# SEP-software/zfp-par

Hardware: AMD Instinct MI355X
Metric: GB/s uncompressed, 3D float32 fixed-rate encode, device-resident (higher is better)
Workload: dtype f32; 1 GPU; 1024^3 float32 fixed-rate 16 zfp_compress per GPU (BASELINE configs[1]); field=smooth, mode=rate, param=16, stream_bytes_per_gpu=2147483648, parallelism=1 independent z-slab chunks, one per GPU

## Files before the change

zfp-par_amd/csrc/hip/block3.h:

```cpp
#pragma once

#include "codec_dev.h"

namespace zfp_amd {

template <typename S>
__device__ __forceinline__ void pad_line(S* v, int b, int s, int n)
{
  if (n <= 1) v[b + s] = v[b];
  if (n <= 2) v[b + 2 * s] = v[b + s];
  if (n <= 3) v[b + 3 * s] = v[b];
}

struct FastDiv {
  uint32_t m, s1, s2;
};

__host__ __device__ inline FastDiv make_fastdiv(uint32_t d)
{
  if (d == 0)
    d = 1;
  uint32_t l = 0;
  while (l < 32 && (1ull << l) < d)
    l++;
// ... 82 lines not shown
#ifndef ZFP_NT_LOAD
#define ZFP_NT_LOAD 1
#endif
#ifndef ZFP_NT_STORE
#define ZFP_NT_STORE 1
#endif
template <typename S, int N>
__device__ __forceinline__ Vec16<S, N> load16(const S* p)
{
#if ZFP_NT_LOAD && defined(__HIP_DEVICE_COMPILE__)
  typedef uint32_t u4 __attribute__((ext_vector_type(4)));
  const u4 x = __builtin_nontemporal_load(reinterpret_cast<const u4*>(p));
  Vec16<S, N> r;
  __builtin_memcpy(&r, &x, 16);
  return r;
#else
  return *reinterpret_cast<const Vec16<S, N>*>(p);
#endif
}

template <typename S, int N>
__device__ __forceinline__ void store16(S* p, const Vec16<S, N>& q)
{
#if ZFP_NT_STORE && defined(__HIP_DEVICE_COMPILE__)
  typedef uint32_t u4 __attribute__((ext_vector_type(4)));
  u4 x;
  __builtin_memcpy(&x, &q, 16);
  __builtin_nontemporal_store(x, reinterpret_cast<u4*>(p));
#else
  *reinterpret_cast<Vec16<S, N>*>(p) = q;
#endif
}

template <typename S, bool VEC, bool NOPART = false>
__device__ __forceinline__ void gather3(S (&v)[64], const S* __restrict__ base, const Geometry& g, const BlockPos& p)
{
  const S* o = base + p.off;
  const int64_t sx = g.s[0], sy = g.s[1], sz = g.s[2];
  if (NOPART || p.full) {
#pragma unroll
    for (int k = 0; k < 4; k++)
#pragma unroll
      for (int j = 0; j < 4; j++) {
        const S* r = o + j * sy + k * sz;
        if (VEC) {
          if constexpr (sizeof(S) == 4) {
            const Vec16<S, 4> q = load16<S, 4>(r);
#pragma unroll
            for (int i = 0; i < 4; i++)
              v[16 * k + 4 * j + i] = q.v[i];
          } else {
            const Vec16<S, 2> q0 = load16<S, 2>(r);
            const Vec16<S, 2> q1 = load16<S, 2>(r + 2);
            v[16 * k + 4 * j + 0] = q0.v[0];
            v[16 * k + 4 * j + 1] = q0.v[1];
            v[16 * k + 4 * j + 2] = q1.v[0];
            v[16 * k + 4 * j + 3] = q1.v[1];
          }
        } else {
#pragma unroll
          for (int i = 0; i < 4; i++)
            v[16 * k + 4 * j + i] = r[i * sx];
        }
      }
  } else {
    const int cx = p.cnt[0], cy = p.cnt[1], cz = p.cnt[2];
#pragma unroll
    for (int k = 0; k < 4; k++)
#pragma unroll
      for (int j = 0; j < 4; j++)
#pragma unroll
        for (int i = 0; i < 4; i++)
          v[16 * k + 4 * j + i] = (i < cx && j < cy && k < cz) ? o[i * sx + j * sy + k * sz] : (S)0;
#pragma unroll
    for (int k = 0; k < 4; k++)
#pragma unroll
      for (int j = 0; j < 4; j++)
        if (k < cz && j < cy) pad_line(v, 16 * k + 4 * j, 1, cx);
#pragma unroll
    for (int k = 0; k < 4; k++)
#pragma unroll
      for (int i = 0; i < 4; i++)
        if (k < cz) pad_line(v, 16 * k + i, 4, cy);
#pragma unroll
    for (int j = 0; j < 4; j++)
#pragma unroll
      for (int i = 0; i < 4; i++)
        pad_line(v, 4 * j + i, 16, cz);
  }
}

template <typename S, bool VEC>
__device__ __forceinline__ void scatter3(const S (&v)[64], S* __restrict__ base, const Geometry& g, const BlockPos& p)
{
  S* o = base + p.off;
  const int64_t sx = g.s[0], sy = g.s[1], sz = g.s[2];
  if (p.full) {
#pragma unroll
    for (int k = 0; k < 4; k++)
#pragma unroll
      for (int j = 0; j < 4; j++) {
        S* r = o + j * sy + k * sz;
        if (VEC) {
          if constexpr (sizeof(S) == 4) {
            Vec16<S, 4> q;
#pragma unroll
            for (int i = 0; i < 4; i++)
              q.v[i] = v[16 * k + 4 * j + i];
            store16<S, 4>(r, q);
          } else {
            Vec16<S, 2> q0, q1;
            q0.v[0] = v[16 * k + 4 * j + 0];
            q0.v[1] = v[16 * k + 4 * j + 1];
            q1.v[0] = v[16 * k + 4 * j + 2];
            q1.v[1] = v[16 * k + 4 * j + 3];
            store16<S, 2>(r, q0);
            store16<S, 2>(r + 2, q1);
          }
        } else {
#pragma unroll
          for (int i = 0; i < 4; i++)
            r[i * sx] = v[16 * k + 4 * j + i];
        }
      }
  } else {
    const int cx = p.cnt[0], cy = p.cnt[1], cz = p.cnt[2];
#pragma unroll
    for (int k = 0; k < 4; k++)
#pragma unroll
      for (int j = 0; j < 4; j++)
#pragma unroll
        for (int i = 0; i < 4; i++)
          if (i < cx && j < cy && k < cz) o[i * sx + j * sy + k * sz] = v[16 * k + 4 * j + i];
  }
}

template <bool P3 = true>
__device__ __forceinline__ void planes_from_coeffs(uint32_t (&Pl)[32], uint32_t (&Ph)[32], const int32_t (&q)[64])
{
#pragma unroll
  for (int i = 0; i < 32; i++) {
    Pl[i] = nb_planes((uint32_t)q[P3 ? kPerm3[i] : i] + 0xaaaaaaaau);
    Ph[i] = nb_planes((uint32_t)q[P3 ? kPerm3[i + 32] : i + 32] + 0xaaaaaaaau);
  }
  transpose32_nb(Pl);
  transpose32_nb(Ph);
}

#ifndef ZFP_NARROW_HI
#define ZFP_NARROW_HI 1
#endif

template <bool P3 = true, int B = 32, int E = 64>
__device__ __forceinline__ bool high_half_narrow(const int32_t (&q)[64])
{
  uint32_t acc = 0;
#pragma unroll
  for (int i = B; i < E; i++)
    acc = __builtin_amdgcn_bitop3_b32(acc, (uint32_t)q[P3 ? kPerm3[i] : i] + 0xaaaaaaaau, 0xaaaaaaaau, 0xf6);
  return acc < 256u;
}

template <bool P3 = true>
__device__ __forceinline__ void planes_high_narrow(uint32_t (&Ph)[32], const int32_t (&q)[64])
{
  uint32_t W[8];
#pragma unroll
  for (int j = 0; j < 8; j++) {
    uint32_t a[4];
#pragma unroll
    for (int b = 0; b < 4; b++)
      a[b] = nb_planes((uint32_t)q[P3 ? kPerm3[32 + 8 * b + j] : 32 + 8 * b + j] + 0xaaaaaaaau);
    const uint32_t t0 = __builtin_amdgcn_perm(a[1], a[0], 0x05010400u);
    const uint32_t t1 = __builtin_amdgcn_perm(a[3], a[2], 0x05010400u);
    W[j] = __builtin_amdgcn_perm(t1, t0, 0x05040100u);
  }
  transpose8x4_nb(W);
#pragma unroll
  for (int k = 0; k < 32; k++)
    Ph[k] = k < 8 ? W[k] : 0u;
}

template <bool P3 = true>
__device__ __forceinline__ void planes_high_full(uint32_t (&Ph)[32], const int32_t (&q)[64])
{
#pragma unroll
  for (int i = 0; i < 32; i++)
    Ph[i] = nb_planes((uint32_t)q[P3 ? kPerm3[i + 32] : i + 32] + 0xaaaaaaaau);
  transpose32_nb(Ph);
}

template <bool P3 = true>
__device__ __forceinline__ void planes_low(uint32_t (&Pl)[32], const int32_t (&q)[64])
{
#pragma unroll
  for (int i = 0; i < 32; i++)
    Pl[i] = nb_planes((uint32_t)q[P3 ? kPerm3[i] : i] + 0xaaaaaaaau);
  transpose32_nb(Pl);
}

template <bool P3 = true>
__device__ __forceinline__ void planes_from_coeffs_narrow(uint32_t (&Pl)[32], uint32_t (&Ph)[32],
                                                          const int32_t (&q)[64])
{
  planes_low<P3>(Pl, q);
  planes_high_narrow<P3>(Ph, q);
}

template <bool P3 = true>
__device__ __forceinline__ void planes_from_coeffs_auto(uint32_t (&Pl)[32], uint32_t (&Ph)[32],
                                                        const int32_t (&q)[64])
{
  planes_low<P3>(Pl, q);
  pin_registers(Pl);
  if (ZFP_NARROW_HI && __builtin_amdgcn_ballot_w64(!high_half_narrow<P3, 32, 40>(q)) == 0 &&
      __builtin_amdgcn_ballot_w64(!high_half_narrow<P3, 40, 64>(q)) == 0)
    planes_high_narrow<P3>(Ph, q);
  else
    planes_high_full<P3>(Ph, q);
}

template <bool P3 = true>
__device__ __forceinline__ void planes_from_coeffs(uint32_t (&Pl)[64], uint32_t (&Ph)[64], const int64_t (&q)[64],
                                                   bool need_low)
{
  uint32_t a[32], b[32];
#pragma unroll
  for (int i = 0; i < 32; i++) {
    uint64_t u0 = nb_planes((uint64_t)q[P3 ? kPerm3[i] : i] + 0xaaaaaaaaaaaaaaaaull);
    uint64_t u1 = nb_planes((uint64_t)q[P3 ? kPerm3[i + 32] : i + 32] + 0xaaaaaaaaaaaaaaaaull);
    a[i] = (uint32_t)(u0 >> 32);
    b[i] = (uint32_t)(u1 >> 32);
  }
  transpose32_nb(a);
  transpose32_nb(b);
#pragma unroll
  for (int k = 0; k < 32; k++) {
    Pl[32 + k] = a[k];
    Ph[32 + k] = b[k];
  }
  if (__any(need_low)) {
#pragma unroll
    for (int i = 0; i < 32; i++) {
      uint64_t u0 = nb_planes((uint64_t)q[P3 ? kPerm3[i] : i] + 0xaaaaaaaaaaaaaaaaull);
      uint64_t u1 = nb_planes((uint64_t)q[P3 ? kPerm3[i + 32] : i + 32] + 0xaaaaaaaaaaaaaaaaull);
      a[i] = (uint32_t)u0;
      b[i] = (uint32_t)u1;
    }
    transpose32_nb(a);
    transpose32_nb(b);
#pragma unroll
    for (int k = 0; k < 32; k++) {
      Pl[k] = a[k];
      Ph[k] = b[k];
    }
  } else {
#pragma unroll
    for (int k = 0; k < 32; k++) {
      Pl[k] = 0;
      Ph[k] = 0;
    }
  }
}

template <bool P3 = true>
__device__ __forceinline__ void coeffs_from_planes(int32_t (&q)[64], const uint64_t (&P)[32])
{
  uint32_t lo[32], hi[32];
#pragma unroll
  for (int k = 0; k < 32; k++) {
    lo[k] = (uint32_t)P[k];
    hi[k] = (uint32_t)(P[k] >> 32);
  }
  transpose32_dnb(lo);
  transpose32_dnb(hi);
#pragma unroll
  for (int i = 0; i < 32; i++) {
    q[P3 ? kPerm3[i] : i] = (int32_t)(lo[i] - 0xaaaaaaaau);
    q[P3 ? kPerm3[i + 32] : i + 32] = (int32_t)(hi[i] - 0xaaaaaaaau);
  }
}

template <bool P3 = true>
__device__ __forceinline__ void coeffs_from_planes(int64_t (&q)[64], const uint64_t (&P)[64], bool need_low)
{
  uint32_t a[32], b[32], c[32], d[32];
#pragma unroll
  for (int k = 0; k < 32; k++) {
    a[k] = (uint32_t)P[32 + k];
    b[k] = (uint32_t)(P[32 + k] >> 32);
  }
  transpose32_dnb(a);
  transpose32_dnb(b);
  if (__any(need_low)) {
#pragma unroll
    for (int k = 0; k < 32; k++) {
      c[k] = (uint32_t)P[k];
      d[k] = (uint32_t)(P[k] >> 32);
    }
    transpose32_dnb(c);
    transpose32_dnb(d);
  } else {
#pragma unroll
    for (int k = 0; k < 32; k++) {
      c[k] = 0xaaaaaaaau;
      d[k] = 0xaaaaaaaau;
    }
  }
#pragma unroll
  for (int i = 0; i < 32; i++) {
    uint64_t u0 = ((uint64_t)a[i] << 32) | c[i];
    uint64_t u1 = ((uint64_t)b[i] << 32) | d[i];
    q[P3 ? kPerm3[i] : i] = (int64_t)(u0 - 0xaaaaaaaaaaaaaaaaull);
    q[P3 ? kPerm3[i + 32] : i + 32] = (int64_t)(u1 - 0xaaaaaaaaaaaaaaaaull);
  }
}

template <bool P3 = true>
__device__ __forceinline__ void planes_hi(uint32_t (&Pl)[32], uint32_t (&Ph)[32], const int64_t (&q)[64])
{
#pragma unroll
  for (int i = 0; i < 32; i++) {
    uint64_t u0 = nb_planes((uint64_t)q[P3 ? kPerm3[i] : i] + 0xaaaaaaaaaaaaaaaaull);
    uint64_t u1 = nb_planes((uint64_t)q[P3 ? kPerm3[i + 32] : i + 32] + 0xaaaaaaaaaaaaaaaaull);
    Pl[i] = (uint32_t)(u0 >> 32);
    Ph[i] = (uint32_t)(u1 >> 32);
  }
  transpose32_nb(Pl);
  transpose32_nb(Ph);
}

template <bool P3 = true>
__device__ __forceinline__ void coeffs_from_planes_hi(int64_t (&q)[64], const uint64_t (&P)[32])
{
  uint32_t a[32], b[32];
#pragma unroll
  for (int k = 0; k < 32; k++) {
    a[k] = (uint32_t)P[k];
    b[k] = (uint32_t)(P[k] >> 32);
  }
  transpose32_dnb(a);
  transpose32_dnb(b);
#pragma unroll
  for (int i = 0; i < 32; i++) {
    q[P3 ? kPerm3[i] : i] = (int64_t)((uint64_t)(a[i] - 0xaaaaaaaau) << 32);
    q[P3 ? kPerm3[i + 32] : i + 32] = (int64_t)((uint64_t)(b[i] - 0xaaaaaaaau) << 32);
  }
}

__device__ __forceinline__ uint32_t precision3(int emax, const CodecParams& cp)
{
  int p = emax - cp.minexp + 2 * 3 + 2;
  if (p < 0) p = 0;
  return (uint32_t)p < cp.maxprec ? (uint32_t)p : cp.maxprec;
}

template <bool PLIM, bool HI = false, typename Int>
__device__ __forceinline__ uint32_t encode_ints3(OrSlot& w, const uint32_t* lut, Int (&q)[64], uint32_t pos,
                                                 uint32_t lim, uint32_t prec)
{
  using S = typename std::conditional<sizeof(Int) == 4, float, double>::type;
  constexpr int PREC = Traits<S>::kIntPrec;
  if constexpr (HI && PREC == 64) {
    uint32_t Pl[32], Ph[32];
    planes_hi(Pl, Ph, q);
    pin_registers(Pl);
    pin_registers(Ph);
    return code_planes<32, PLIM>(w, lut, pos, lim, prec, Pl, Ph);
  } else {
    uint32_t Pl[PREC], Ph[PREC];
    if constexpr (PREC == 32)
      planes_from_coeffs(Pl, Ph, q);
    else
      planes_from_coeffs(Pl, Ph, q, prec > 32);
    pin_registers(Pl);
    pin_registers(Ph);
    return code_planes<PREC, PLIM>(w, lut, pos, lim, prec, Pl, Ph);
  }
}

template <bool HI = false, typename Int>
__device__ __forceinline__ uint32_t decode_ints3(WordReader& r, const uint32_t* sq, Int (&q)[64], uint32_t budget,
                                                 uint32_t prec)
{
  using S = typename std::conditional<sizeof(Int) == 4, float, double>::type;
  constexpr int PREC = Traits<S>::kIntPrec;
  if constexpr (HI && PREC == 64) {
    uint64_t P[32];
    const uint32_t used = decode_planes32<false>(r, sq, budget, prec, P);
    pin_registers(P);
    coeffs_from_planes_hi(q, P);
    return used;
  } else {
    uint64_t P[PREC];
    uint32_t used;
    if constexpr (PREC == 32)
      used = decode_planes32(r, sq, budget, prec, P);
    else
      used = decode_planes64<PREC>(r, sq, budget, prec, P);
    pin_registers(P);
    if constexpr (PREC == 32)
      coeffs_from_planes(q, P);
    else
      coeffs_from_planes(q, P, prec > 32);
    return used;
  }
}

template <typename Reload>
__device__ __forceinline__ int lossy_emax_cast(int32_t (&q)[64], float (&v)[64], const CodecParams& cp,
                                               uint32_t& mp, Reload&& reload)
{
  int32_t mi = 0;
  uint32_t mu = 0;
#pragma unroll
  for (int i = 0; i < 64; i++) {
    const uint32_t b = __float_as_uint(v[i]);
    mi = max(mi, (int32_t)b);
    mu = max(mu, b);
  }
  const uint32_t mb = max((uint32_t)mi, mu & 0x7fffffffu);
  int emax = mb == 0 ? -127 : ((mb >> 23) == 0 ? -126 : (int)(mb >> 23) - 126);
  const bool bad = mb >= 0x7f800000u;
  if (bad)
    emax = block_emax(block_absmax(v));
  mp = precision3(emax, cp);
  const bool cast = mp != 0 && emax != -127;
  const float s = __uint_as_float((uint32_t)(157 - emax) << 23);
#pragma unroll
  for (int i = 0; i < 64; i++)
    q[i] = (int32_t)(s * v[i]);
  if (__any(cast && (bad || emax < -97))) {
    float w[64];
    reload(w);
    fwd_cast(q, w, emax);
  }
  return emax;
}

template <typename Reload>
__device__ __forceinline__ int lossy_emax_cast(int64_t (&q)[64], double (&v)[64], const CodecParams& cp,
                                               uint32_t& mp, Reload&&)
{
  const int emax = block_emax(block_absmax(v));
  mp = precision3(emax, cp);
  fwd_cast(q, v, emax);
  return emax;
}

#if defined(__HIP_DEVICE_COMPILE__)
#define ZFP_PHASE_BARRIER() __builtin_amdgcn_sched_barrier(0)
#else
#define ZFP_PHASE_BARRIER() ((void)0)
#endif

template <bool NARROW = false, typename S, typename Reload, typename Mid>
__device__ __forceinline__ void encode_block3_fixed(OrSlot& w, const uint32_t* lut, S (&v)[64], const CodecParams& cp,
                                                    Reload&& reload, Mid&& mid)
{
  using T = Traits<S>;
  using Int = typename T::Int;
  constexpr int PREC = T::kIntPrec;
  constexpr uint32_t kE = T::kEbits;
  Int q[64];
  uint32_t mp;
  const int emax = lossy_emax_cast(q, v, cp, mp, reload);
  const uint32_t e = mp ? (uint32_t)(emax + T::kEbias) : 0u;
  if (e)
    w.head(2 * e + 1);
  ZFP_PHASE_BARRIER();
  xform<3, false, false>(q);
  ZFP_PHASE_BARRIER();
  uint32_t Pl[PREC], Ph[PREC];
  if constexpr (PREC == 32) {
    if constexpr (NARROW)
      planes_from_coeffs_auto(Pl, Ph, q);
    else
      planes_from_coeffs(Pl, Ph, q);
    ZFP_PHASE_BARRIER();
    pin_registers(Pl);
    pin_registers(Ph);
    mid();
    code_planes_fr32(w.d(), w.jmax, lut, e ? 1 + kE : cp.maxbits, cp.maxbits, Pl, Ph);
  } else {
    planes_from_coeffs(Pl, Ph, q, true);
    ZFP_PHASE_BARRIER();
    pin_registers(Pl);
    pin_registers(Ph);
    mid();
    code_planes<PREC, false>(w, lut, e ? 1 + kE : cp.maxbits, cp.maxbits, mp, Pl, Ph);
  }
}

template <typename S, bool REV, bool FR = false, bool HI = false, bool NARROW = false, typename Reload>
__device__ __forceinline__ uint32_t encode_block3(OrSlot& w, const uint32_t* lut, S (&v)[64], const CodecParams& cp,
                                                  Reload&& reload)
{
  using T = Traits<S>;
  using Int = typename T::Int;
  using UInt = typename T::UInt;
  constexpr uint32_t kE = T::kEbits;
  Int q[64];
  if constexpr (REV) {
    int emax = block_emax(block_absmax(v));
    decltype(bits_of(v[0])) sdiff = 0;
    bool same;
    if (emax != -T::kEbias) {
      fwd_cast(q, v, emax);
      S s = (sizeof(S) == 4) ? (S)pow2f(emax - 30) : (S)pow2d(emax - 62);
#pragma unroll
      for (int i = 0; i < 64; i++) {
        sdiff |= bits_of((S)(s * (S)q[i])) ^ bits_of(v[i]);
        if ((i & 3) == 3)
          pin_value(sdiff);
      }
    } else {
#pragma unroll
      for (int i = 0; i < 64; i++) {
        q[i] = 0;
        sdiff |= bits_of(v[i]);
      }
    }
    same = sdiff == 0;
    uint32_t bits;
    if (same) {
      uint32_t e = (uint32_t)(emax + T::kEbias);
      if (!e) {
        return 1u < cp.minbits ? cp.minbits : 1u;
      }
      w.head(1u | (e << 2));
      bits = 2 + kE;
    } else {
#pragma unroll
      for (int i = 0; i < 64; i++) {
        const Int x = (Int)bits_of(v[i]);
        q[i] = x < 0 ? (Int)((UInt)x ^ T::kTcMask) : x;
        if ((i & 3) == 3)
          ZFP_SCHED_FENCE();
      }
      w.head(3u);
      bits = 2;
    }
    const uint32_t minb = cp.minbits - (bits < cp.minbits ? bits : cp.minbits);
    xform<3, false, true>(q);
    UInt all = 0;
#pragma unroll
    for (int i = 0; i < 64; i++)
      all |= ((UInt)q[i] + T::kNbMask) ^ T::kNbMask;
    uint32_t prec = all ? (uint32_t)(T::kIntPrec - (sizeof(S) == 4 ? __builtin_ctz((uint32_t)all)
                                                                    : __builtin_ctzll((uint64_t)all)))
                        : 0u;
    if (prec > cp.maxprec) prec = cp.maxprec;
    if (prec < 1) prec = 1;
    w.put32(bits, prec - 1);
    const uint32_t end = encode_ints3<true, HI>(w, lut, q, bits + T::kPbits, cp.maxbits, prec);
    uint32_t ib = end - bits;
    if (ib < minb) ib = minb;
    return bits + ib;
  } else {
    if constexpr (FR && !HI) {
      encode_block3_fixed<NARROW>(w, lut, v, cp, reload, [] {});
      return cp.maxbits;
    }
    uint32_t mp;
    const int emax = lossy_emax_cast(q, v, cp, mp, reload);
    const uint32_t e = mp ? (uint32_t)(emax + T::kEbias) : 0u;
    uint32_t bits = 1;
    if (e) {
      w.head(2 * e + 1);
      bits += kE;
      xform<3, false, false>(q);
      const uint32_t minb = cp.minbits - (bits < cp.minbits ? bits : cp.minbits);
      uint32_t ib = encode_ints3<!FR, HI>(w, lut, q, bits, cp.maxbits, mp) - bits;
      if (ib < minb) ib = minb;
      bits += ib;
    } else if (cp.minbits > bits) {
      bits = cp.minbits;
    }
    return bits;
  }
}

template <typename S, bool REV, bool HI = false>
__device__ __forceinline__ uint32_t decode_block3(WordReader& r, const uint32_t* sq, S (&v)[64], const CodecParams& cp)
{
  using T = Traits<S>;
  using Int = typename T::Int;
  using UInt = typename T::UInt;
  constexpr uint32_t kE = T::kEbits;
  Int q[64];
  if constexpr (REV) {
    uint32_t bits = 1;
    if (!r.read1()) {
#pragma unroll
      for (int i = 0; i < 64; i++) v[i] = 0;
      if (cp.minbits > bits) {
        r.skip(cp.minbits - bits);
        bits = cp.minbits;
      }
      return bits;
    }
    bits++;
    bool reinterp = r.read1() != 0;
    int emax = 0;
    if (!reinterp) {
      bits += kE;
      emax = (int)r.read(kE) - T::kEbias;
    }
    uint32_t minb = cp.minbits - (bits < cp.minbits ? bits : cp.minbits);
    uint32_t maxb = cp.maxbits - bits;
    uint32_t prec = (uint32_t)r.read(T::kPbits) + 1;
    uint32_t ib = T::kPbits + decode_ints3<HI>(r, sq, q, maxb - T::kPbits, prec);
    if (ib < minb) {
      r.skip(minb - ib);
      ib = minb;
    }
    xform<3, true, true>(q);
    if (reinterp) {
#pragma unroll
      for (int i = 0; i < 64; i++) {
        Int x = q[i] < 0 ? (Int)((UInt)q[i] ^ T::kTcMask) : q[i];
        if constexpr (sizeof(S) == 4)
          v[i] = __uint_as_float((uint32_t)x);
        else
          v[i] = __longlong_as_double((long long)x);
      }
    } else if (emax != -T::kEbias) {
      inv_cast(v, q, emax);
    } else {
#pragma unroll
      for (int i = 0; i < 64; i++) v[i] = 0;
    }
    return bits + ib;
  } else {
  uint32_t bits = 1;
  if (r.read1()) {
    bits += kE;
    int emax = (int)r.read(kE) - T::kEbias;
    uint32_t mp = precision3(emax, cp);
    uint32_t minb = cp.minbits - (bits < cp.minbits ? bits : cp.minbits);
    uint32_t ib = decode_ints3<HI>(r, sq, q, cp.maxbits - bits, mp);
    if (ib < minb) {
      r.skip(minb - ib);
      ib = minb;
    }
    bits += ib;
    xform<3, true, false>(q);
// ... 15 lines not shown
```

zfp-par_amd/csrc/hip/codec_dev.h:

```cpp
#pragma once

#include <hip/hip_runtime.h>
#include <stdint.h>

#include "zfp_perm_dev.h"

namespace zfp_amd {

constexpr int kMinExp = -1074;

template <typename S>
struct Traits;

template <>
struct Traits<float> {
  using Int = int32_t;
  using UInt = uint32_t;
  static constexpr int kEbits = 8;
  static constexpr int kPbits = 5;
  static constexpr int kEbias = 127;
  static constexpr int kIntPrec = 32;
  static constexpr UInt kNbMask = 0xaaaaaaaau;
  static constexpr UInt kTcMask = 0x7fffffffu;
};
// ... 597 lines not shown
    if ((PLIM || k < ZFP_FR_EXIT_PLANES) && __builtin_amdgcn_ballot_w64(act) == 0)
      break;
    const uint32_t pl = Pl[k], ph = Ph[k];
    const uint32_t Nl = pl & ~Sl, Nh = ph & ~Sh;
    const uint64_t N = ((uint64_t)Nh << 32) | Nl;
    const bool nz = N != 0;
    const uint32_t clz = (uint32_t)__clzll((long long)(N | 1ull));
    const uint32_t n1 = nz ? 64u - clz : n;
    const uint64_t S1 = nz ? (~0ull >> clz) : (((uint64_t)Sh << 32) | Sl);
    const uint32_t t2 = (uint32_t)__popc(Nh) + ((uint32_t)__popc(Nl) + n1);
    const uint32_t impl = SIZE == 64 ? Nh >> 31 : (uint32_t)(N >> (SIZE - 1)) & 1u;
    const uint64_t xs = N >> (n & 63u);
    const uint32_t x0 = (uint32_t)xs;
    const uint32_t b0 = x0 & 0xffu;
    const uint32_t sh1 = 8u + (uint32_t)__popc(b0);
    const uint32_t l0 = lut[b0], l1 = lut[(x0 >> 8) & 0xffu];
    const uint32_t m = (2u | impl) << ((t2 + nn) & 31u);
    const uint32_t h = n1 + nn;
    const bool ext = SIZE > 16 && act && nz && h >= 16u;
    const int32_t dlen = SIZE == 64 ? (int32_t)t2 + 1 + ((int32_t)(uint32_t)(S1 >> 32) >> 31) + ((int32_t)Nh >> 31)
                                    : (int32_t)t2 + 1 - (int32_t)((S1 >> (SIZE - 1)) & 1u) - (int32_t)impl;
    if (!PLIM) {
      uint32_t* q = dm1 + opaque_shr5(p31);
      const uint32_t t = 31u - p31;
      const uint32_t v0 = pl ^ Nl, v1 = ph ^ Nh;
      lds_or32(q, __builtin_amdgcn_alignbit(v0, 0u, t));
      lds_or32(q + 1, __builtin_amdgcn_alignbit(v1, v0, t));
      lds_or32(q + 2, __builtin_amdgcn_alignbit(0u, v1, t));
    }
    if (__builtin_amdgcn_ballot_w64(ext) != 0) {
      const uint32_t g32 = (l1 << sh1) >> 31;
      const ExtEvent e{p31 - 31u + n, x0, (uint32_t)(xs >> 32), h | (impl << 6) | (g32 << 7)};
      if constexpr (PREC <= 32) {
        expand_event(s, lut, ExtEvent{e.gp, e.xl, e.xh, ext ? e.hb : 0u});
      } else if (ext) {
        e2 = e1;
        e1 = e0;
        e0 = e;
      }
    }
    const uint32_t d16 = l0 | (l1 << sh1);
    const uint32_t g = ((d16 << 1) | (nz ? 1u : 0u)) - (ext ? 0u : m);
    if (PLIM) {
      if (act) {
        s.put64_clamped(p31 - 31u, pl ^ Nl, ph ^ Nh);
        s.put32_clamped(p31 - 31u + n, g);
      }
      p31 = act ? p31 + (uint32_t)dlen : p31;
      n = act ? n1 : n;
      Sl = act ? (uint32_t)S1 : Sl;
      Sh = act ? (uint32_t)(S1 >> 32) : Sh;
    } else {
      const uint32_t pg = p31 + n;
      uint32_t* q = dm1 + opaque_shr5(pg);
      const uint32_t t = 31u - pg;
      lds_or32(q, __builtin_amdgcn_alignbit(g, 0u, t));
      lds_or32(q + 1, __builtin_amdgcn_alignbit(0u, g, t));
      p31 += (uint32_t)dlen;
      p31 = p31 < lim31 ? p31 : lim31;
      n = n1;
      Sl = (uint32_t)S1;
      Sh = (uint32_t)(S1 >> 32);
    }
    nn = ~n;
  }
  if constexpr (PREC > 32) {
    if (__any(e0.hb >= 16u)) {
      expand_event(s, lut, e0);
      if (__any(e1.hb >= 16u)) {
        expand_event(s, lut, e1);
        if (__any(e2.hb >= 16u))
          expand_event(s, lut, e2);
      }
    }
  }
  const uint32_t end = p31 - 31u;
  return end < lim ? end : lim;
}

__device__ __forceinline__ void fr_write32(int32_t Q, uint32_t v)
{
  const uint32_t a = ~(((uint32_t)(Q >> 3)) | 3u);
  ZFP_LDS_OR(lds_at(a), __builtin_amdgcn_alignbit(v, 0u, (uint32_t)Q));
  ZFP_LDS_OR(lds_at(a + 4u), __builtin_amdgcn_alignbit(0u, v, (uint32_t)Q));
}

__device__ __forceinline__ void fr_write64(int32_t Q, uint32_t v0, uint32_t v1)
{
  const uint32_t a = ~(((uint32_t)(Q >> 3)) | 3u);
  ZFP_LDS_OR(lds_at(a), __builtin_amdgcn_alignbit(v0, 0u, (uint32_t)Q));
  ZFP_LDS_OR(lds_at(a + 4u), __builtin_amdgcn_alignbit(v1, v0, (uint32_t)Q));
  ZFP_LDS_OR(lds_at(a + 8u), __builtin_amdgcn_alignbit(0u, v1, (uint32_t)Q));
}

#ifndef ZFP_FR32
#define ZFP_FR32 1
#endif
#ifndef ZFP_FRU
#define ZFP_FRU 1
#endif

__device__ __forceinline__ void code_planes_fru(OrSlot& os, const uint32_t* lut, uint32_t sb, int32_t Q,
                                                int32_t Qlim, uint32_t n, int kstart, const uint32_t (&Pl)[32],
                                                const uint32_t (&Ph)[32])
{
  const uint32_t tdbl = lds_off(lut), tlead = tdbl + 1024u;
  uint32_t Sh = n > 32u ? ~0u >> ((0u - n) & 31u) : 0u;
#pragma unroll
  for (int k = 31; k >= 0; k--) {
    if (k > kstart)
      continue;
    if (k < ZFP_FR_EXIT_PLANES && __builtin_amdgcn_ballot_w64(Q > Qlim) == 0)
      break;
    exp_vpad();
    const uint32_t pl = Pl[k], ph = Ph[k];
    const bool hi = n >= 32u;
    const uint32_t Nh = ph & ~Sh;
    const uint32_t t = Nh >> (n & 31u);
    const uint32_t x0 = hi ? t : __builtin_amdgcn_alignbit(Nh, pl, n);
    const uint32_t x1 = hi ? 0u : t;
    const uint32_t l0 = *lds_at(tlead + byte0_x4(x0));
    const uint32_t l1 = *lds_at(tdbl + byte1_x4(x0));
    const uint32_t bl = 31u - (uint32_t)__clz((int)((x0 << 1) | 1u));
    const uint32_t e1 = (uint32_t)__popc(x0) + bl;
    const uint32_t impl = Nh >> 31;
    uint32_t n1 = n + bl;
    const uint32_t d = (l1 << (l0 & 31u)) | (l0 >> 5);
    uint32_t g = ubfe(d, 0u, e1 - impl);
    uint32_t L = e1 - impl + 1u - (n1 >> 6);
    const bool ext = x0 > 0xfffeu || x1 != 0u;
    const int32_t Qg = Q - (int32_t)n;
    if (__builtin_amdgcn_ballot_w64(ext) != 0) {
      uint32_t hb = 0;
      if (ext) {
        const uint32_t hx = x1 ? 63u - (uint32_t)__clz((int)x1) : 31u - (uint32_t)__clz((int)x0);
        const uint32_t c = (uint32_t)__popc(x0) + (uint32_t)__popc(x1);
        n1 = n + hx + 1u;
        const uint32_t im = n1 >> 6;
        L = hx + c + 2u - 2u * im;
        g = hx < 16u ? d & ~(im << 31) : d;
        hb = hx | (im << 6) | ((x0 & 0xffffu) == 0xffffu ? 0x80u : 0u);
      }
      expand_event(os, lut, ExtEvent{(uint32_t)(-Qg) - sb, x0, x1, hb});
    }
    fr_write64(Q, hi ? pl : ubfe(pl, 0u, n), ph & Sh);
    fr_write32(Qg, g);
    const int32_t Qn = Qg - (int32_t)L;
    Q = Qn > Qlim ? Qn : Qlim;
    n = n1;
    Sh = n > 32u ? ~0u >> ((0u - n) & 31u) : 0u;
  }
}

__device__ __forceinline__ void code_planes_fr32(uint32_t* slot, uint32_t jmax, const uint32_t* lut, uint32_t pos,
                                                 uint32_t lim, const uint32_t (&Pl)[32], const uint32_t (&Ph)[32])
{
  OrSlot os{reinterpret_cast<uint64_t*>(slot), jmax};
#if ZFP_FR32
  const uint32_t sb = lds_off(slot) * 8u;
  const uint32_t tdbl = lds_off(lut), tlead = tdbl + 1024u;
  int32_t Q = -(int32_t)(sb + pos);
  const int32_t Qlim = -(int32_t)(sb + lim);
  uint32_t n = 0;
  bool m32 = true;
  int ksw = 0;
#pragma unroll
  for (int k = 31; k >= 0; k--) {
    if (m32) {
      if (__builtin_amdgcn_ballot_w64(Ph[k] != 0u || n > 31u) != 0) {
        m32 = false;
        ksw = k;
      } else {
        exp_vpad();
        const uint32_t pl = Pl[k];
        const uint32_t xs = pl >> n;
        const uint32_t l0 = *lds_at(tlead + byte0_x4(xs));
        const uint32_t l1 = *lds_at(tdbl + byte1_x4(xs));
        const uint32_t bl = 32u - (uint32_t)__clz((int)xs);
        const uint32_t e1 = (uint32_t)__popc(xs) + bl;
        if (k != 31)
          fr_write32(Q, ubfe(pl, 0u, n));
        const int32_t Qg = Q - (int32_t)n;
        const uint32_t d = (l1 << (l0 & 31u)) | (l0 >> 5);
        uint32_t g = d - (1u << (e1 & 31u));
        const bool ext = xs > 0xfffeu;
        if (__builtin_amdgcn_ballot_w64(ext) != 0) {
          const uint32_t h = 31u - (uint32_t)__clz((int)xs);
          const uint32_t gp = (uint32_t)(-Qg) - sb;
          const uint32_t g32 = (xs & 0xffffu) == 0xffffu ? 1u : 0u;
          g = ext ? d : g;
          expand_event(os, lut, ExtEvent{gp, xs, 0u, ext ? h | (g32 << 7) : 0u});
        }
        fr_write32(Qg, g);
        const int32_t Qn = Qg - (int32_t)e1 - 1;
        Q = Qn > Qlim ? Qn : Qlim;
        n += bl;
      }
    }
  }
  if (!m32) {
#if ZFP_FRU
    code_planes_fru(os, lut, sb, Q, Qlim, n, ksw, Pl, Ph);
#else
    code_planes<32, false>(os, lut, (uint32_t)(-Q) - sb, lim, 32u, Pl, Ph, ksw, n);
#endif
  }
#else
  code_planes<32, false>(os, lut, pos, lim, 32u, Pl, Ph);
#endif
}

constexpr uint64_t kEven = 0x5555555555555555ull;
constexpr uint64_t kOdd = 0xaaaaaaaaaaaaaaaaull;

__device__ __forceinline__ uint32_t squeeze_entry(uint32_t b)
{
  uint32_t o = 0, r = 0;
#pragma unroll
  for (int l = 0; l < 8; l++) {
    if ((b >> l) & 1u) {
      o |= 1u << (l - r);
      r++;
    }
  }
  return o;
}

template <int SIZE = 64>
__device__ __forceinline__ void decode_group_slow(WordReader& r, uint64_t& x, uint32_t& bits, uint32_t& n)
{
  while (bits && n < (uint32_t)SIZE) {
    bits--;
    if (!r.read1())
      break;
    uint32_t lim = (uint32_t)SIZE - 1 - n;
    if (lim > bits)
      lim = bits;
    uint32_t z = ctz64(r.peek64());
    if (z < lim) {
      r.skip(z + 1);
      bits -= z + 1;
      n += z;
    } else {
      r.skip(lim);
      bits -= lim;
      n += lim;
    }
    x |= 1ull << n;
    n++;
  }
}

__device__ __forceinline__ uint32_t squeeze32(const uint32_t* sq, uint32_t f)
{
  const uint32_t b0 = f & 0xffu, b1 = (f >> 8) & 0xffu, b2 = (f >> 16) & 0xffu, b3 = f >> 24;
  const uint32_t u0 = sq[b0] | (sq[b1] << (8u - (uint32_t)__popc(b0)));
  const uint32_t u1 = sq[b2] | (sq[b3] << (8u - (uint32_t)__popc(b2)));
  return u0 | (u1 << (16u - (uint32_t)__popc(f & 0xffffu)));
}

template <bool IMP = true, int SIZE = 64>
__device__ __forceinline__ uint64_t decode_plane64(WordReader& r, const uint32_t* sq, uint32_t& bits, uint32_t& n)
{
  const uint32_t m = n < bits ? n : bits;
  uint32_t pos = r.pos;
  const uint64_t V = r.peek_at(pos);
  uint64_t x = m ? V & (~0ull >> ((64u - m) & 63u)) : 0ull;
  pos += m;
  uint32_t bl = bits - m;
  const bool grp = n < (uint32_t)SIZE && bl != 0;
  if (!__any(grp)) {
    r.pos = pos;
    bits = bl;
    return x;
  }
  const uint64_t w = r.peek_at(pos);
  const bool one = (w & 1) != 0;
  const uint64_t S = w >> 1;
  const uint64_t starts = S & ~(S << 1);
  const uint64_t se = S + (starts & kEven), so = S + (starts & kOdd);
  const uint64_t ends = (((se & ~S) & kOdd) | ((so & ~S) & kEven)) & ~(1ull << 63);
  const uint32_t q = ctz64(ends);
  const uint64_t mq = (ends - 1) & ~ends;
  const uint32_t ones = (uint32_t)__popcll(S & mq);
  const uint32_t P = q - (ones - 1) / 2;
  const bool fast = grp && one && ends != 0 && n + P <= (uint32_t)SIZE - 1 && q + 2 <= bl;
  const bool imp0 = IMP && grp && one && !fast && (ends == 0 || n + P > (uint32_t)SIZE - 1);
  const uint64_t F = (fast || imp0) ? S & mq & (((S & ~se) & kEven) | ((S & ~so) & kOdd)) : 0ull;
  const uint32_t Fl = (uint32_t)F, Fh = (uint32_t)(F >> 32);
  uint64_t xx = squeeze32(sq, Fl);
  if (ZFP_RARE(__any(Fh != 0)))
    xx |= (uint64_t)squeeze32(sq, Fh) << (32u - (uint32_t)__popc(Fl));
  uint32_t k63 = 0, si = 0;
  uint64_t xi = 0;
  bool imp = false;
  if (ZFP_RARE(__any(imp0))) {
    k63 = ((uint32_t)SIZE - 1 - n) & 63u;
    xi = xx & ((1ull << k63) - 1);
    si = k63 + (uint32_t)__popcll(xi);
    imp = imp0 && si <= 63u && si + 1u <= bl;
  }
  x |= (fast ? xx : (imp ? xi | (1ull << k63) : 0ull)) << (n & 63u);
  const uint32_t used = fast ? q + 2u : (imp ? si + 1u : (grp && !one ? 1u : 0u));
  n = fast ? n + P : (imp ? (uint32_t)SIZE : n);
  r.pos = pos + used;
  bits = bl - used;
// ... 132 lines not shown
```

zfp-par_amd/csrc/hip/kernels3.h:

```cpp
#pragma once

#include "block3.h"
#include "blockn.h"

namespace zfp_amd {

constexpr int kWavesPerGroup = 4;
constexpr size_t kLutBytes = 256 * sizeof(uint32_t);
constexpr uint64_t kNoWord = ~0ull;

struct Partial {
  uint64_t idx;
  uint64_t val;
};

__device__ __forceinline__ uint32_t wave_incl_scan(uint32_t x)
{
  const int lane = (int)lane_id_fresh();
#pragma unroll
  for (int d = 1; d < 64; d <<= 1) {
    uint32_t y = __shfl_up(x, d, 64);
    if (lane >= d) x += y;
  }
  return x;
// ... 47 lines not shown
    for (uint32_t i = lane; i < 16 * sdw; i += 64)
      z[i] = make_uint4(0, 0, 0, 0);
    __builtin_amdgcn_s_waitcnt(0xc07f);
    __builtin_amdgcn_wave_barrier();
  }
  if (b < g.nblocks) {
    OrSlot os{reinterpret_cast<uint64_t*>(wslot + (size_t)lane * sdw), sdw - 1};
    encode_block3<S, REV, true, false, true>(os, lut, v, cp, [&](S (&r)[64]) { gather3<S, VEC>(r, data, g, p); });
  }
  if (first >= g.nblocks)
    return;
  __builtin_amdgcn_fence(__ATOMIC_SEQ_CST, "wavefront");
  __builtin_amdgcn_wave_barrier();
  const uint64_t nb = (g.nblocks - first) < 64 ? (g.nblocks - first) : 64;
  const uint32_t total = (uint32_t)nb * sw;
  uint64_t* dst = out + first * sw;
  auto run_word = [&](uint32_t i) -> uint64_t {
    const uint32_t l = div_magic(i, magic_w);
    const uint32_t* s = wslot + (size_t)l * sdw + 2 * (i - l * sw);
    return (uint64_t)s[0] | ((uint64_t)s[1] << 32);
  };
  if (r0 == 0) {
    if ((sw & 1) == 0) {
      const uint32_t hw = sw >> 1, chunks = (uint32_t)nb * hw;
      for (uint32_t c = lane; c < chunks; c += 64) {
        const uint32_t l = div_magic(c, magic_c);
        const uint32_t* s = wslot + (size_t)l * sdw + 4 * (c - l * hw);
#if ZFP_NT_STORE && defined(__HIP_DEVICE_COMPILE__)
        typedef uint32_t u4 __attribute__((ext_vector_type(4)));
        __builtin_nontemporal_store(u4{s[0], s[1], s[2], s[3]}, reinterpret_cast<u4*>(dst + 2 * c));
#else
        *reinterpret_cast<uint4*>(dst + 2 * c) = make_uint4(s[0], s[1], s[2], s[3]);
#endif
      }
    } else {
      for (uint32_t i = lane; i < total; i += 64)
        dst[i] = run_word(i);
    }
    return;
  }
  if ((sw & 1) == 0) {
    const uint32_t hw = sw >> 1, chunks = (uint32_t)nb * hw;
    const uint32_t jj = (r0 + 31u) >> 5, sh = 32u * jj - r0;
    const uint32_t o0 = (uint32_t)(reinterpret_cast<uintptr_t>(dst) >> 3) & 1u;
    for (uint32_t c = lane; c < chunks; c += 64) {
      const uint32_t l = div_magic(c, magic_c), cs = c - l * hw;
      const uint32_t* s = wslot + (size_t)l * sdw + 4 * cs;
      uint32_t X[6];
      if (o0 == 0) {
        const uint32_t* q = cs ? s - 2 : wslot + (size_t)(l ? l - 1 : 0) * sdw + 2 * sw - 2;
        X[0] = c ? q[0] : 0u;
        X[1] = c ? q[1] : 0u;
        X[2] = s[0], X[3] = s[1], X[4] = s[2], X[5] = s[3];
      } else {
        const bool in_run = 2 * c + 2 < total;
        const uint32_t* q = cs + 1 < hw ? s + 4 : wslot + (size_t)(in_run ? l + 1 : l) * sdw;
        X[0] = s[0], X[1] = s[1], X[2] = s[2], X[3] = s[3];
        X[4] = in_run ? q[0] : 0u;
        X[5] = in_run ? q[1] : 0u;
      }
      uint32_t y[4];
#pragma unroll
      for (int i = 0; i < 4; i++)
        y[i] = jj == 1 ? __builtin_amdgcn_alignbit(X[i + 2], X[i + 1], sh) : __builtin_amdgcn_alignbit(X[i + 1], X[i], sh);
      const uint32_t o = o0 + 2 * c;
      const uint64_t v0 = ((uint64_t)y[1] << 32) | y[0], v1 = ((uint64_t)y[3] << 32) | y[2];
      if (o == 0) {
        partials[2 * w] = Partial{first * sw, v0};
        dst[1] = v1;
      } else if (o + 1 == total) {
        dst[o] = v0;
        partials[2 * w + 1] = Partial{first * sw + total, v1};
      } else {
#if ZFP_NT_STORE && defined(__HIP_DEVICE_COMPILE__)
        typedef uint32_t u4 __attribute__((ext_vector_type(4)));
        __builtin_nontemporal_store(u4{y[0], y[1], y[2], y[3]}, reinterpret_cast<u4*>(dst + o));
#else
        *reinterpret_cast<uint4*>(dst + o) = make_uint4(y[0], y[1], y[2], y[3]);
#endif
      }
    }
    if (lane == 0) {
      if (o0 == 0)
        partials[2 * w + 1] = Partial{first * sw + total, run_word(total - 1) >> (64 - r0)};
      else
        partials[2 * w] = Partial{first * sw, run_word(0) << r0};
    }
    return;
  }
  for (uint32_t j = lane; j <= total; j += 64) {
    const uint64_t cur = j < total ? run_word(j) : 0ull;
    const uint64_t prev = j > 0 ? run_word(j - 1) : 0ull;
    const uint64_t val = (cur << r0) | (prev >> (64 - r0));
    if (j == 0) {
      partials[2 * w] = Partial{first * sw, val};
    } else if (j == total) {
      partials[2 * w + 1] = Partial{first * sw + total, val};
    } else {
      dst[j] = val;
    }
  }
}

template <int SW>
constexpr uint32_t kAlignedSlotDwords = slot_dwords_for(64u * SW) | 1u;

template <typename S, bool VEC, bool NOPART = false, int SW = 0>
__global__ __launch_bounds__(256, 3) void encode3_aligned_full(const S* __restrict__ data, Geometry g, CodecParams cp,
                                                            uint64_t* __restrict__ out, uint32_t sw_, uint32_t sdw_,
                                                            uint32_t magic_c)
{
  constexpr uint32_t kHw = SW / 2;
  static_assert(SW == 0 || (SW % 2 == 0 && kHw <= 64 && (kHw & (kHw - 1)) == 0), "SW: 2 hw, hw a power of two");
  const uint32_t sw = SW ? (uint32_t)SW : sw_;
  const uint32_t sdw = SW ? kAlignedSlotDwords<SW> : sdw_;
  __shared__ uint32_t lut[512];
  extern __shared__ uint32_t ldsw[];
  const int lane = threadIdx.x & 63;
  const int wv = NOPART ? __builtin_amdgcn_readfirstlane((int)(threadIdx.x >> 6)) : (int)(threadIdx.x >> 6);
  uint32_t* wslot = ldsw + (size_t)wv * 64 * sdw;
  const uint64_t w = (uint64_t)blockIdx.x * kWavesPerGroup + wv;
  const uint64_t first = w * 64;
  const uint64_t b = first + lane;
  S v[64];
  __builtin_amdgcn_s_setprio(1);
  BlockPos p;
  if (NOPART && (g.nb[0] & 63u) == 0)
    p = block_pos_row3(g, (uint32_t)first, (uint32_t)lane);
  else
    p = block_pos<NOPART>(g, b, 3);
  gather3<S, VEC, NOPART>(v, data, g, p);
  __builtin_amdgcn_s_setprio(0);
  {
    const uint4* src = reinterpret_cast<const uint4*>(&kCoderTables);
    uint4* dst = reinterpret_cast<uint4*>(lut);
    dst[lane] = src[lane];
    dst[lane + 64] = src[lane + 64];
    uint4* z = reinterpret_cast<uint4*>(wslot);
    if constexpr (SW != 0) {
      constexpr uint32_t kQuads = 16 * kAlignedSlotDwords<SW>;
#pragma unroll
      for (uint32_t i = 0; i < kQuads / 64; i++)
        z[lane + 64 * i] = make_uint4(0, 0, 0, 0);
      if (kQuads % 64 != 0 && (uint32_t)lane < kQuads % 64)
        z[lane + (kQuads & ~63u)] = make_uint4(0, 0, 0, 0);
    } else {
      for (uint32_t i = lane; i < 16 * sdw; i += 64)
        z[i] = make_uint4(0, 0, 0, 0);
    }
    __builtin_amdgcn_s_waitcnt(0xc07f);
    __builtin_amdgcn_wave_barrier();
  }
  OrSlot os{reinterpret_cast<uint64_t*>(wslot + (size_t)lane * sdw), sdw - 1};
  encode_block3<S, false, true, false, NOPART>(os, lut, v, cp,
                                               [&](S (&r)[64]) { gather3<S, VEC, NOPART>(r, data, g, p); });
  __builtin_amdgcn_fence(__ATOMIC_SEQ_CST, "wavefront");
  __builtin_amdgcn_wave_barrier();
  uint64_t* dst = out + first * sw;
  if constexpr (SW != 0) {
    const uint32_t ln = (uint32_t)lane;
    const uint32_t* s = wslot + (ln / kHw) * sdw + 4 * (ln % kHw);
    uint64_t* d = dst + 2 * ln;
    uint32_t r[kHw][4];
#pragma unroll
    for (uint32_t i = 0; i < kHw; i++)
#pragma unroll
      for (int j = 0; j < 4; j++)
        r[i][j] = s[i * (64 / kHw) * sdw + j];
#pragma unroll
    for (uint32_t i = 0; i < kHw; i++) {
#if ZFP_NT_STORE && defined(__HIP_DEVICE_COMPILE__)
      typedef uint32_t u4 __attribute__((ext_vector_type(4)));
      __builtin_nontemporal_store(u4{r[i][0], r[i][1], r[i][2], r[i][3]}, reinterpret_cast<u4*>(d + 128 * i));
#else
      *reinterpret_cast<uint4*>(d + 128 * i) = make_uint4(r[i][0], r[i][1], r[i][2], r[i][3]);
#endif
    }
  } else {
    const uint32_t hw = sw >> 1, chunks = 64 * hw;
    for (uint32_t c = lane; c < chunks; c += 64) {
      const uint32_t l = div_magic(c, magic_c);
      const uint32_t* s = wslot + (size_t)l * sdw + 4 * (c - l * hw);
#if ZFP_NT_STORE && defined(__HIP_DEVICE_COMPILE__)
      typedef uint32_t u4 __attribute__((ext_vector_type(4)));
      __builtin_nontemporal_store(u4{s[0], s[1], s[2], s[3]}, reinterpret_cast<u4*>(dst + 2 * c));
#else
      *reinterpret_cast<uint4*>(dst + 2 * c) = make_uint4(s[0], s[1], s[2], s[3]);
#endif
    }
  }
  __builtin_amdgcn_s_waitcnt(0x0f70);
}

__device__ __forceinline__ uint64_t slot_bits(const uint64_t* slot, uint32_t pos, uint32_t cnt)
{
  uint32_t i = pos >> 6, r = pos & 63;
  uint64_t v = slot[i] >> r;
  if (r && r + cnt > 64)
    v |= slot[i + 1] << (64 - r);
  return v & low_mask(cnt);
}

__device__ __forceinline__ uint64_t slot_bits_l2(uint64_t* slot, uint32_t pos, uint32_t cnt)
{
  uint32_t i = pos >> 6, r = pos & 63;
  uint64_t v = __hip_atomic_load(slot + i, __ATOMIC_RELAXED, __HIP_MEMORY_SCOPE_AGENT) >> r;
  if (r && r + cnt > 64)
    v |= __hip_atomic_load(slot + i + 1, __ATOMIC_RELAXED, __HIP_MEMORY_SCOPE_AGENT) << (64 - r);
  return v & low_mask(cnt);
}

struct GeneralArgs {
  uint64_t* out;
  uint32_t g0;
  uint32_t swp;
  uint32_t var;
  uint32_t maxbits;
  uint64_t* status;
  uint32_t* ticket;
  Partial* partials;
  uint16_t* idx_len;
  uint64_t* idx_base;
  uint64_t* total_bits;
  uint32_t* error;
  uint64_t idx_add;
  uint64_t* ovf;
  uint32_t* ovf_count;
  uint32_t ovf_cap;
  uint32_t ovf_swp;
  uint32_t cap_bits;
#ifdef ZFP_EXP4_TRACE
  uint64_t* trace;
#endif
};

constexpr uint32_t kNoSlot = ~0u;

__device__ __forceinline__ uint32_t take_overflow_slot(const GeneralArgs& a)
{
  uint32_t oi = atomicAdd(a.ovf_count, 1u);
  if (oi >= a.ovf_cap) {
    atomicOr(a.error, 2u);
    oi = kNoSlot;
  }
  return oi;
}

__device__ __forceinline__ void zero_words(uint64_t* p, uint32_t n)
{
  for (uint32_t i = 0; i < n; i++)
    p[i] = 0;
}

constexpr uint64_t kStAgg = 1ull << 62;
constexpr uint64_t kStIncl = 2ull << 62;
constexpr uint64_t kStMask = (1ull << 62) - 1;


__device__ __forceinline__ uint64_t lookback_lane(uint64_t* status, uint64_t w, uint32_t agg, uint32_t* error)
{
  uint64_t excl = 0;
  if (w == 0) {
    __hip_atomic_store(&status[0], kStIncl | agg, __ATOMIC_RELAXED, __HIP_MEMORY_SCOPE_AGENT);
    return 0;
  }
  __hip_atomic_store(&status[w], kStAgg | agg, __ATOMIC_RELAXED, __HIP_MEMORY_SCOPE_AGENT);
  uint64_t j = w - 1;
  uint32_t spins = 0;
  for (;;) {
    const uint64_t st = __hip_atomic_load(&status[j], __ATOMIC_RELAXED, __HIP_MEMORY_SCOPE_AGENT);
    const uint64_t tag = st & ~kStMask;
    if (tag == 0) {
      if (++spins > (1u << 26)) {
        atomicOr(error, 1u);
        break;
      }
      __builtin_amdgcn_s_sleep(1);
      continue;
    }
    excl += st & kStMask;
    if (tag == kStIncl || j == 0)
      break;
    j--;
  }
  __hip_atomic_store(&status[w], kStIncl | (excl + agg), __ATOMIC_RELAXED, __HIP_MEMORY_SCOPE_AGENT);
  return excl;
}

__device__ __forceinline__ uint64_t wave_sum64(uint64_t x)
{
#pragma unroll
  for (int d = 1; d < 64; d <<= 1)
    x += __shfl_xor(x, d, 64);
  return x;
}

__device__ __forceinline__ void lookback_publish(uint64_t* status, uint64_t w, uint32_t agg)
{
  if (lane_id_fresh() == 0)
    __hip_atomic_store(&status[w], (w == 0 ? kStIncl : kStAgg) | agg, __ATOMIC_RELAXED, __HIP_MEMORY_SCOPE_AGENT);
}

__device__ __forceinline__ uint64_t lookback_walk(uint64_t* status, uint64_t w, uint32_t agg, uint32_t* error)
{
  const uint32_t lane = lane_id_fresh();
  if (w == 0)
    return 0;
  uint64_t excl = 0;
// ... 412 lines not shown
```

Before: 3609 GB/s.

## Precompute wave-uniform plane classes to skip empty and low-density bit planes

When the high half of a block's coefficients is narrow, the encoder now computes, across the wave, the highest nonzero plane (ksw) and the plane below which group tests are needed (kS). It then calls a specialized fixed-rate 32-bit plane coder that skips planes above ksw in groups of four and uses a simpler no-extension path for dense planes. The aim is to remove per-plane ballot checks and wasted work on empty top planes for smooth data. It adds a DPP wave reduction, an extra code-path instantiation with more code size and register pressure, and a fallback to the general coder when the classification is not computed.

After: 3702 GB/s (median of 6 runs). 1.03x the previous value.

```diff
diff --git a/zfp-par_amd/csrc/hip/block3.h b/zfp-par_amd/csrc/hip/block3.h
--- a/zfp-par_amd/csrc/hip/block3.h
+++ b/zfp-par_amd/csrc/hip/block3.h
@@ -258,13 +258,18 @@
 #endif
 
 template <bool P3 = true, int B = 32, int E = 64>
-__device__ __forceinline__ bool high_half_narrow(const int32_t (&q)[64])
-{
-  uint32_t acc = 0;
+__device__ __forceinline__ uint32_t nb_or(const int32_t (&q)[64], uint32_t acc = 0)
+{
 #pragma unroll
   for (int i = B; i < E; i++)
     acc = __builtin_amdgcn_bitop3_b32(acc, (uint32_t)q[P3 ? kPerm3[i] : i] + 0xaaaaaaaau, 0xaaaaaaaau, 0xf6);
-  return acc < 256u;
+  return acc;
+}
+
+template <bool P3 = true, int B = 32, int E = 64>
+__device__ __forceinline__ bool high_half_narrow(const int32_t (&q)[64])
+{
+  return nb_or<P3, B, E>(q) < 256u;
 }
 
 template <bool P3 = true>
@@ -313,17 +318,41 @@
   planes_high_narrow<P3>(Ph, q);
 }
 
-template <bool P3 = true>
-__device__ __forceinline__ void planes_from_coeffs_auto(uint32_t (&Pl)[32], uint32_t (&Ph)[32],
-                                                        const int32_t (&q)[64])
+template <bool P3 = true, bool CLS = false>
+__device__ __forceinline__ PlaneClass planes_from_coeffs_auto(uint32_t (&Pl)[32], uint32_t (&Ph)[32],
+                                                              const int32_t (&q)[64])
 {
   planes_low<P3>(Pl, q);
   pin_registers(Pl);
-  if (ZFP_NARROW_HI && __builtin_amdgcn_ballot_w64(!high_half_narrow<P3, 32, 40>(q)) == 0 &&
-      __builtin_amdgcn_ballot_w64(!high_half_narrow<P3, 40, 64>(q)) == 0)
+  uint32_t a = 0;
+  bool narrow = false;
+  if (ZFP_NARROW_HI) {
+    a = nb_or<P3, 32, 40>(q);
+    if (__builtin_amdgcn_ballot_w64(a >= 256u) == 0) {
+      a = nb_or<P3, 40, 64>(q, a);
+      narrow = __builtin_amdgcn_ballot_w64(a >= 256u) == 0;
+    }
+  }
+  PlaneClass pc{kPlanesTested, 32};
+  if (narrow) {
+    if constexpr (CLS) {
+      const uint32_t b = ((uint32_t)q[P3 ? kPerm3[31] : 31] + 0xaaaaaaaau) ^ 0xaaaaaaaau;
+      pc.ksw = (int)nbits32(wave_or(a | (b >> 1))) - 1;
+      pc.kS = 0;
+#pragma unroll
+      for (int k = 31; k >= 0; k--) {
+        if (__builtin_amdgcn_ballot_w64(Pl[k] > 0x7fffu) != 0) {
+          pc.kS = k + 1;
+          break;
+        }
+      }
+      pc.kS = pc.kS > pc.ksw ? pc.kS : pc.ksw + 1;
+    }
     planes_high_narrow<P3>(Ph, q);
-  else
+  } else {
     planes_high_full<P3>(Ph, q);
+  }
+  return pc;
 }
 
 template <bool P3 = true>
@@ -560,7 +589,7 @@
 #define ZFP_PHASE_BARRIER() ((void)0)
 #endif
 
-template <bool NARROW = false, typename S, typename Reload, typename Mid>
+template <int NARROW = 0, typename S, typename Reload, typename Mid>
 __device__ __forceinline__ void encode_block3_fixed(OrSlot& w, const uint32_t* lut, S (&v)[64], const CodecParams& cp,
                                                     Reload&& reload, Mid&& mid)
 {
@@ -579,15 +608,19 @@
   ZFP_PHASE_BARRIER();
   uint32_t Pl[PREC], Ph[PREC];
   if constexpr (PREC == 32) {
-    if constexpr (NARROW)
-      planes_from_coeffs_auto(Pl, Ph, q);
+    PlaneClass pc{kPlanesTested, 32};
+    if constexpr (NARROW != 0)
+      pc = planes_from_coeffs_auto<true, NARROW == 2>(Pl, Ph, q);
     else
       planes_from_coeffs(Pl, Ph, q);
     ZFP_PHASE_BARRIER();
     pin_registers(Pl);
     pin_registers(Ph);
     mid();
-    code_planes_fr32(w.d(), w.jmax, lut, e ? 1 + kE : cp.maxbits, cp.maxbits, Pl, Ph);
+    if (NARROW == 2 && pc.ksw != kPlanesTested)
+      code_planes_fr32(w.d(), w.jmax, lut, e ? 1 + kE : cp.maxbits, cp.maxbits, Pl, Ph, pc);
+    else
+      code_planes_fr32(w.d(), w.jmax, lut, e ? 1 + kE : cp.maxbits, cp.maxbits, Pl, Ph);
   } else {
     planes_from_coeffs(Pl, Ph, q, true);
     ZFP_PHASE_BARRIER();
@@ -598,7 +631,7 @@
   }
 }
 
-template <typename S, bool REV, bool FR = false, bool HI = false, bool NARROW = false, typename Reload>
+template <typename S, bool REV, bool FR = false, bool HI = false, int NARROW = 0, typename Reload>
 __device__ __forceinline__ uint32_t encode_block3(OrSlot& w, const uint32_t* lut, S (&v)[64], const CodecParams& cp,
                                                   Reload&& reload)
 {
diff --git a/zfp-par_amd/csrc/hip/codec_dev.h b/zfp-par_amd/csrc/hip/codec_dev.h
--- a/zfp-par_amd/csrc/hip/codec_dev.h
+++ b/zfp-par_amd/csrc/hip/codec_dev.h
@@ -773,6 +773,105 @@
   }
 }
 
+#ifndef ZFP_PLANE_CLASS
+#define ZFP_PLANE_CLASS 1
+#endif
+constexpr int kPlanesTested = -2;
+struct PlaneClass {
+  int ksw;
+  int kS;
+};
+
+__device__ __forceinline__ uint32_t nbits32(uint32_t x) { return 32u - (uint32_t)__clz((int)x); }
+
+__device__ __forceinline__ uint32_t wave_or(uint32_t x)
+{
+#ifdef __HIP_DEVICE_COMPILE__
+  int v = (int)x;
+  v |= __builtin_amdgcn_update_dpp(0, v, 0x111, 0xf, 0xf, true);
+  v |= __builtin_amdgcn_update_dpp(0, v, 0x112, 0xf, 0xf, true);
+  v |= __builtin_amdgcn_update_dpp(0, v, 0x114, 0xf, 0xf, true);
+  v |= __builtin_amdgcn_update_dpp(0, v, 0x118, 0xf, 0xf, true);
+  v |= __builtin_amdgcn_update_dpp(0, v, 0x142, 0xa, 0xf, false);
+  v |= __builtin_amdgcn_update_dpp(0, v, 0x143, 0xc, 0xf, false);
+  return (uint32_t)__builtin_amdgcn_readlane(v, 63);
+#else
+  return x;
+#endif
+}
+
+__device__ __forceinline__ void code_planes_fr32(uint32_t* slot, uint32_t jmax, const uint32_t* lut, uint32_t pos,
+                                                 uint32_t lim, const uint32_t (&Pl)[32], const uint32_t (&Ph)[32],
+                                                 const PlaneClass& pc)
+{
+  OrSlot os{reinterpret_cast<uint64_t*>(slot), jmax};
+#if ZFP_FR32
+  const uint32_t sb = lds_off(slot) * 8u;
+  const uint32_t tdbl = lds_off(lut), tlead = tdbl + 1024u;
+  int32_t Q = -(int32_t)(sb + pos);
+  const int32_t Qlim = -(int32_t)(sb + lim);
+  const int ksw = pc.ksw, kS = pc.kS;
+  uint32_t n = 0;
+#pragma unroll
+  for (int k4 = 28; k4 >= 0; k4 -= 4) {
+    if (ksw >= k4 + 3)
+      continue;
+#pragma unroll
+    for (int k = k4 + 3; k >= k4; k--) {
+      if (k >= kS) {
+        exp_vpad();
+        const uint32_t pl = Pl[k];
+        const uint32_t xs = k == 31 ? pl : pl >> n;
+        const uint32_t l0 = *lds_at(tlead + byte0_x4(xs));
+        const uint32_t l1 = *lds_at(tdbl + byte1_x4(xs));
+        const uint32_t n1 = (k == 31 ? 0u : n) + nbits32(xs);
+        const uint32_t ne = (uint32_t)__popc(xs) + n1;
+        const uint32_t d = (l1 << (l0 & 31u)) | (l0 >> 5);
+        const uint32_t v = k == 31 ? d - (1u << (ne & 31u)) : pl + ((d - xs) << n) - (1u << (ne & 31u));
+        fr_write32(Q, v);
+        const int32_t Qn = Q - (int32_t)ne - 1;
+        Q = Qn > Qlim ? Qn : Qlim;
+        n = n1;
+      } else if (k > ksw) {
+        exp_vpad();
+        const uint32_t pl = Pl[k];
+        const uint32_t xs = pl >> n;
+        const uint32_t l0 = *lds_at(tlead + byte0_x4(xs));
+        const uint32_t l1 = *lds_at(tdbl + byte1_x4(xs));
+        const uint32_t bl = nbits32(xs);
+        const uint32_t e1 = (uint32_t)__popc(xs) + bl;
+        if (k != 31)
+          fr_write32(Q, ubfe(pl, 0u, n));
+        const int32_t Qg = Q - (int32_t)n;
+        const uint32_t d = (l1 << (l0 & 31u)) | (l0 >> 5);
+        uint32_t g = d - (1u << (e1 & 31u));
+        const bool ext = xs > 0xfffeu;
+        if (__builtin_amdgcn_ballot_w64(ext) != 0) {
+          const uint32_t h = 31u - (uint32_t)__clz((int)xs);
+          const uint32_t gp = (uint32_t)(-Qg) - sb;
+          const uint32_t g32 = (xs & 0xffffu) == 0xffffu ? 1u : 0u;
+          g = ext ? d : g;
+          expand_event(os, lut, ExtEvent{gp, xs, 0u, ext ? h | (g32 << 7) : 0u});
+        }
+        fr_write32(Qg, g);
+        const int32_t Qn = Qg - (int32_t)e1 - 1;
+        Q = Qn > Qlim ? Qn : Qlim;
+        n += bl;
+      }
+    }
+  }
+  if (ksw >= 0) {
+#if ZFP_FRU
+    code_planes_fru(os, lut, sb, Q, Qlim, n, ksw, Pl, Ph);
+#else
+    code_planes<32, false>(os, lut, (uint32_t)(-Q) - sb, lim, 32u, Pl, Ph, ksw, n);
+#endif
+  }
+#else
+  code_planes<32, false>(os, lut, pos, lim, 32u, Pl, Ph);
+#endif
+}
+
 __device__ __forceinline__ void code_planes_fr32(uint32_t* slot, uint32_t jmax, const uint32_t* lut, uint32_t pos,
                                                  uint32_t lim, const uint32_t (&Pl)[32], const uint32_t (&Ph)[32])
 {
diff --git a/zfp-par_amd/csrc/hip/kernels3.h b/zfp-par_amd/csrc/hip/kernels3.h
--- a/zfp-par_amd/csrc/hip/kernels3.h
+++ b/zfp-par_amd/csrc/hip/kernels3.h
@@ -223,8 +223,8 @@
     __builtin_amdgcn_wave_barrier();
   }
   OrSlot os{reinterpret_cast<uint64_t*>(wslot + (size_t)lane * sdw), sdw - 1};
-  encode_block3<S, false, true, false, NOPART>(os, lut, v, cp,
-                                               [&](S (&r)[64]) { gather3<S, VEC, NOPART>(r, data, g, p); });
+  encode_block3<S, false, true, false, NOPART ? 1 + ZFP_PLANE_CLASS : 0>(
+    os, lut, v, cp, [&](S (&r)[64]) { gather3<S, VEC, NOPART>(r, data, g, p); });
   __builtin_amdgcn_fence(__ATOMIC_SEQ_CST, "wavefront");
   __builtin_amdgcn_wave_barrier();
   uint64_t* dst = out + first * sw;
```
